# XUANTIE-RV/csi-nn2

Measured on AMD Instinct MI355X. Metric: mobilenetv1_int8_images_per_sec, higher is better.
Workload: dtype i8; 1 GPU; mobilenetv1 int8 NHWC batch 1/GPU, 28 conv layers in 15 launches, hipGraph replay via csinn_*; ops_per_image=1137480704, algorithmic_bytes_per_image=8323144, algorithmic_bytes_per_image_survey=14444616, parallelism=replicas x1

## Files before the change

csi-nn2_amd/csrc/conv1x1_latency.hip:

```cpp
#include <stdlib.h>

#include "igemm_common.h"

namespace shl {

struct LatPoolArgs {
    void *out;
    float si, zi, so, zo;
    int32_t store_map;
};

template <int NSW, int MT, int EPI, bool POOL>
__global__ __launch_bounds__(512) void conv1x1_latency_kernel(ConvArgs a, LatPoolArgs pl)
{
    extern __shared__ __attribute__((aligned(16))) char smem[];
    asm volatile("" ::"s"(a.in), "s"(a.w_frag), "s"(a.out), "s"(a.acc_init), "s"(a.mult), "s"(a.bias), "s"(a.C), "s"(a.Co), "s"(a.Ho), "s"(a.Wo));
    const int tid = threadIdx.x;
    const int lane = tid & 63;
    const int wave = __builtin_amdgcn_readfirstlane(tid >> 6);
    const int frow = lane & 31, fhalf = lane >> 5;
    const int slice = blockIdx.x, n = blockIdx.y;
    const int t0 = blockIdx.z;
    const int HW = a.Ho * a.Wo;
    constexpr int NSUB = 8 * NSW;
    const int sub0 = wave * NSW;

    const char *wp = static_cast<const char *>(a.w_frag) + ((int64_t)slice * NSUB + sub0) * 1024 + lane * 16;
    v4i fa[NSW];
#pragma unroll
    for (int s = 0; s < NSW; ++s) fa[s] = *reinterpret_cast<const v4i *>(wp + s * 1024);
    const char *img = static_cast<const char *>(a.in) + (int64_t)n * HW * a.C + fhalf * 16 + sub0 * 32;
    v4i fb[MT][NSW];
#pragma unroll
    for (int t = 0; t < MT; ++t) {
        const int p = min((t0 + t) * 32 + frow, HW - 1);
        const char *px = img + p * a.C;
#pragma unroll
        for (int s = 0; s < NSW; ++s) fb[t][s] = *reinterpret_cast<const v4i *>(px + s * 32);
    }
    const int fgrp = wave & 3, ftile = wave >> 2;
    const int pc = slice * 32 + 8 * fgrp + 4 * fhalf;
    const int4 p_ai = *reinterpret_cast<const int4 *>(a.acc_init + pc);
    const float4 p_mu = *reinterpret_cast<const float4 *>(a.mult + pc);
    const float4 p_bi = *reinterpret_cast<const float4 *>(a.bias + pc);

    const v16i zero16 = {0, 0, 0, 0, 0, 0, 0, 0, 0, 0, 0, 0, 0, 0, 0, 0};
    v16i acc[MT];
#pragma unroll
    for (int s = 0; s < NSW; ++s)
#pragma unroll
        for (int t = 0; t < MT; ++t) acc[t] = __builtin_amdgcn_mfma_i32_32x32x32_i8(fa[s], fb[t][s], s == 0 ? zero16 : acc[t], 0, 0, 0);

    v4i *part = reinterpret_cast<v4i *>(smem);
#pragma unroll
    for (int t = 0; t < MT; ++t)
#pragma unroll
        for (int g = 0; g < 4; ++g) {
            v4i v;
#pragma unroll
            for (int e = 0; e < 4; ++e) v[e] = acc[t][4 * g + e];
            part[((t * 8 + wave) * 4 + g) * 64 + lane] = v;
        }
    __syncthreads();
    uint32_t *pmap = reinterpret_cast<uint32_t *>(smem + (size_t)MT * 8 * 4096);
    if (ftile < MT) {
        v4i v = part[((ftile * 8) * 4 + fgrp) * 64 + lane];
#pragma unroll
        for (int k = 1; k < 8; ++k) v += part[((ftile * 8 + k) * 4 + fgrp) * 64 + lane];
        const uint32_t pk = requant4_i8_sel<EPI>(v[0] + p_ai.x, v[1] + p_ai.y, v[2] + p_ai.z, v[3] + p_ai.w, p_mu, p_bi, a);
        const int p = (t0 + ftile) * 32 + frow;
        if (p < HW) {
            if (!POOL || pl.store_map) *reinterpret_cast<uint32_t *>(static_cast<char *>(a.out) + ((int64_t)n * HW + p) * a.Co + pc) = pk;
            if constexpr (POOL) pmap[p * 8 + 2 * fgrp + fhalf] = pk;
        }
    }
    if constexpr (POOL) {
        __syncthreads();
        if (tid < 32) {
            const int8_t *col = reinterpret_cast<const int8_t *>(pmap) + tid;
            float total = 0.f;
            for (int p = 0; p < HW; ++p) total = __fadd_rn(total, __fmul_rn(__fsub_rn((float)col[p * 32], pl.zi), pl.si));
            const int q = sat8_from_float(__fadd_rn(rintf(__fdiv_rn(__fdiv_rn(total, (float)HW), pl.so)), pl.zo));
            static_cast<int8_t *>(pl.out)[(int64_t)n * a.Co + slice * 32 + tid] = (int8_t)q;
        }
    }
}

static int lat_epi(const ConvArgs &a) { return (a.act != SHL_MI355X_ACT_NONE && !a.act_clamp) ? -1 : (a.div_exact ? 3 : 0); }

static bool lat_shape(const ConvArgs &a)
{
    if (a.Kh != 1 || a.Kw != 1 || a.sh != 1 || a.sw != 1 || a.pt != 0 || a.pl != 0 || a.H != a.Ho || a.W != a.Wo) return false;
    if (a.C != 256 && a.C != 512 && a.C != 1024) return false;
    if ((a.Co & 31) != 0 || a.kstride < a.C || a.out_nchw || a.in_nchw || !a.w_frag) return false;
    const int HW = a.Ho * a.Wo;
    return HW >= 1 && HW <= 64 && a.N >= 1 && a.N <= 65535 && (a.Co >> 5) <= 65535;
}

bool conv1x1_latency_pick(const ConvArgs &a)
{
    if (!lat_shape(a)) return false;
    const char *env = getenv("SHL_MI355X_PWLAT");
    if (env && env[0] == '0') return false;
    if (env && env[0] == '1') return true;
    return (int64_t)(a.Co >> 5) * a.N <= 256;
}

bool conv1x1_pool_fusable(const ConvArgs &a) { return lat_shape(a) && (int64_t)(a.Co >> 5) * a.N <= 512; }

static int launch_lat(const ConvArgs &a, const LatPoolArgs &pl, hipStream_t s)
{
    const int HW = a.Ho * a.Wo, nsw = a.C / 256, epi = lat_epi(a);
    const bool pool = pl.out != nullptr;
    int mt = HW > 32 ? 2 : 1, zsplit = 1;
    const char *sp = getenv("SHL_MI355X_PWLAT_SPLIT");
    if (!pool && mt == 2 && (int64_t)(a.Co >> 5) * a.N * 2 <= 256 && !(sp && sp[0] == '0')) mt = 1, zsplit = 2;
    const dim3 grid((unsigned)(a.Co >> 5), (unsigned)a.N, (unsigned)zsplit);
    const size_t lds = (size_t)mt * 8 * 4096 + (pool ? (size_t)HW * 32 : 0);
#define SHL_LAT4(NSWV, MTV, EPIV, POOLV)                                                                      \
    do {                                                                                                      \
        static LdsOptIn opted;                                                                                \
        if (lds > 64 * 1024) lds_opt_in(opted, reinterpret_cast<const void *>(conv1x1_latency_kernel<NSWV, MTV, EPIV, POOLV>)); \
        hipLaunchKernelGGL((conv1x1_latency_kernel<NSWV, MTV, EPIV, POOLV>), grid, dim3(512), lds, s, a, pl);     \
    } while (0)
#define SHL_LAT3(NSWV, MTV, EPIV)             \
    do {                                      \
        if (pool) SHL_LAT4(NSWV, MTV, EPIV, true); \
        else SHL_LAT4(NSWV, MTV, EPIV, false);     \
    } while (0)
#define SHL_LAT2(NSWV, MTV)                    \
    do {                                       \
        if (epi == 3) SHL_LAT3(NSWV, MTV, 3);  \
        else if (epi == 0) SHL_LAT3(NSWV, MTV, 0); \
        else SHL_LAT3(NSWV, MTV, -1);          \
    } while (0)
#define SHL_LAT1(NSWV)               \
    do {                             \
        if (mt == 2) SHL_LAT2(NSWV, 2); \
        else SHL_LAT2(NSWV, 1);      \
    } while (0)
    if (nsw == 4) SHL_LAT1(4);
    else if (nsw == 2) SHL_LAT1(2);
    else SHL_LAT1(1);
#undef SHL_LAT1
#undef SHL_LAT2
#undef SHL_LAT3
#undef SHL_LAT4
    SHL_HIP(hipGetLastError());
    return SHL_MI355X_OK;
}

int launch_conv1x1_latency(const ConvArgs &a, hipStream_t s)
{
    if (!lat_shape(a)) {
        set_error("conv1x1_latency: the layer does not qualify");
        return SHL_MI355X_ENOTSUP;
    }
    LatPoolArgs pl = {};
    return launch_lat(a, pl, s);
}

int launch_conv1x1_pool(const ConvArgs &a, void *pool_out, float si, float zi, float so, float zo, int store_map, hipStream_t s)
{
    if (!conv1x1_pool_fusable(a) || !pool_out) {
        set_error("conv1x1_pool: the pair does not qualify");
        return SHL_MI355X_ENOTSUP;
// ... 8 lines not shown
```

csi-nn2_amd/csrc/conv_gemv.hip:

```cpp
#include <stdlib.h>

#include "common.h"

namespace shl {

constexpr int GEMV_OPW = 4;

template <bool kI8, int OPW>
__global__ __launch_bounds__(256) void conv_gemv_kernel(ConvArgs a)
{
    constexpr int ESIZE = kI8 ? 1 : 2;
    const int lane = threadIdx.x & 63;
    const int wave = __builtin_amdgcn_readfirstlane(threadIdx.x >> 6);
    const int p = blockIdx.y;
    const int oc0 = (blockIdx.x * 4 + wave) * OPW;
    if (oc0 >= a.Co) return;
    const int kb = a.C * ESIZE;
    const char *in = static_cast<const char *>(a.in) + (int64_t)p * kb;
    const char *w = static_cast<const char *>(a.w);
    int32_t acc_i[OPW];
    float acc_f[OPW];
#pragma unroll
    for (int o = 0; o < OPW; ++o) acc_i[o] = 0, acc_f[o] = 0.f;
    for (int off = lane * 16; off < kb; off += 1024) {
        const v4i x = *reinterpret_cast<const v4i *>(in + off);
        v4i wv[OPW];
#pragma unroll
        for (int o = 0; o < OPW; ++o) {
            const int oc = oc0 + o < a.Co ? oc0 + o : a.Co - 1;
            wv[o] = *reinterpret_cast<const v4i *>(w + (int64_t)oc * a.kstride + off);
        }
#pragma unroll
        for (int o = 0; o < OPW; ++o)
#pragma unroll
            for (int d = 0; d < 4; ++d) {
                if constexpr (kI8) {
                    acc_i[o] = __builtin_amdgcn_sdot4(x[d], wv[o][d], acc_i[o], false);
                } else {
                    const uint32_t xu = (uint32_t)x[d], wu = (uint32_t)wv[o][d];
                    acc_f[o] += f16_bits_to_float((uint16_t)(xu & 0xffffu)) * f16_bits_to_float((uint16_t)(wu & 0xffffu));
                    acc_f[o] += f16_bits_to_float((uint16_t)(xu >> 16)) * f16_bits_to_float((uint16_t)(wu >> 16));
                }
            }
    }
#pragma unroll
    for (int o = 0; o < OPW; ++o)
#pragma unroll
        for (int s = 32; s >= 1; s >>= 1) {
            if constexpr (kI8)
                acc_i[o] += __shfl_xor(acc_i[o], s, 64);
            else
                acc_f[o] += __shfl_xor(acc_f[o], s, 64);
        }
    if (lane < OPW && oc0 + lane < a.Co) {
        const int oc = oc0 + lane;
        int32_t S = acc_i[0];
        float F = acc_f[0];
#pragma unroll
        for (int o = 1; o < OPW; ++o) S = lane == o ? acc_i[o] : S, F = lane == o ? acc_f[o] : F;
        if constexpr (kI8) {
            static_cast<int8_t *>(a.out)[(int64_t)p * a.Co + oc] =
                (int8_t)requant_i8_fast(S + a.acc_init[oc], a.mult[oc], a.bias[oc], a);
        } else {
            static_cast<uint16_t *>(a.out)[(int64_t)p * a.Co + oc] = finish_f16(F, a.bias[oc], a);
        }
    }
}

constexpr int PG_WAVES = 16;

template <int QMAX>
__global__ __launch_bounds__(PG_WAVES * 64) void pool_gemv_i8_kernel(ConvArgs a, int HW, float si, float zi, float so, float zo)
{
    extern __shared__ __attribute__((aligned(16))) char x_lds[];
    const int tid = threadIdx.x, lane = tid & 63;
    const int wave = __builtin_amdgcn_readfirstlane(tid >> 6);
    const int p = blockIdx.y;
    const int oc0 = (blockIdx.x * PG_WAVES + wave) * GEMV_OPW;
    const bool live = oc0 < a.Co;
    const int kb = a.C;
    const char *w = static_cast<const char *>(a.w);
    v4i wv0[GEMV_OPW];
    {
        const int off = lane * 16;
#pragma unroll
        for (int o = 0; o < GEMV_OPW; ++o) {
            const int oc = oc0 + o < a.Co ? oc0 + o : a.Co - 1;
            wv0[o] = v4i{0, 0, 0, 0};
            if (off < kb) wv0[o] = *reinterpret_cast<const v4i *>(w + (int64_t)oc * a.kstride + off);
        }
    }
    const int row_b = a.C;
    const __amdgpu_buffer_rsrc_t img = __builtin_amdgcn_make_buffer_rsrc(
        const_cast<char *>(static_cast<const char *>(a.in) + (int64_t)p * HW * row_b), 0, HW * row_b, 0x00020000);
    for (int c = tid; c < a.C; c += PG_WAVES * 64) {
        uint32_t v[QMAX];
#pragma unroll
        for (int q = 0; q < QMAX; ++q) {
            const int qq = q < HW ? q : HW - 1;
            v[q] = (uint32_t)__builtin_amdgcn_raw_buffer_load_b32(img, c & ~3, qq * row_b, 0);
        }
        const int sh = 8 * (c & 3);
        float total = 0.f;
#pragma unroll
        for (int q = 0; q < QMAX; ++q) {
            const float x = __fmul_rn(__fsub_rn((float)(int8_t)(v[q] >> sh), zi), si);
            const float t = __fadd_rn(total, x);
            total = q < HW ? t : total;
        }
        x_lds[c] = (char)sat8_from_float(__fadd_rn(rintf(__fdiv_rn(__fdiv_rn(total, (float)HW), so)), zo));
    }
    __syncthreads();
    if (!live) return;
    int32_t acc_i[GEMV_OPW] = {0, 0, 0, 0};
    for (int off = lane * 16; off < kb; off += 1024) {
        const v4i x = *reinterpret_cast<const v4i *>(x_lds + off);
        v4i wv[GEMV_OPW];
#pragma unroll
        for (int o = 0; o < GEMV_OPW; ++o) {
            if (off < 1024) {
                wv[o] = wv0[o];
            } else {
                const int oc = oc0 + o < a.Co ? oc0 + o : a.Co - 1;
                wv[o] = *reinterpret_cast<const v4i *>(w + (int64_t)oc * a.kstride + off);
            }
        }
#pragma unroll
        for (int o = 0; o < GEMV_OPW; ++o)
#pragma unroll
            for (int d = 0; d < 4; ++d) acc_i[o] = __builtin_amdgcn_sdot4(x[d], wv[o][d], acc_i[o], false);
    }
#pragma unroll
    for (int o = 0; o < GEMV_OPW; ++o)
#pragma unroll
        for (int s = 32; s >= 1; s >>= 1) acc_i[o] += __shfl_xor(acc_i[o], s, 64);
    if (lane < GEMV_OPW && oc0 + lane < a.Co) {
        const int oc = oc0 + lane;
        const int32_t S = lane == 0 ? acc_i[0] : lane == 1 ? acc_i[1] : lane == 2 ? acc_i[2] : acc_i[3];
        static_cast<int8_t *>(a.out)[(int64_t)p * a.Co + oc] = (int8_t)requant_i8_fast(S + a.acc_init[oc], a.mult[oc], a.bias[oc], a);
    }
}

bool pool_gemv_pick(const ConvArgs &a, int hw)
{
    return conv_gemv_pick(a, 1) && a.H * a.W == 1 && hw >= 1 && hw <= 64 && a.C % 16 == 0 && a.C <= 32768 && (int64_t)hw * a.C < (1ll << 31);
}

// ... 36 lines not shown
```

csi-nn2_amd/csrc/dw_patch.h:

```cpp
#pragma once

#include "common.h"

namespace shl {

__device__ __forceinline__ int dw_patch_slot(int j, int group, int pitch) { return group * pitch + j; }
__host__ __device__ __forceinline__ int dw_patch_pitch(int npx) { return ((npx + 31) & ~31) + 8; }
__host__ __device__ __forceinline__ size_t dw_patch_bytes(int npx) { return (size_t)dw_patch_pitch(npx) * 32; }
__device__ __forceinline__ uint32_t dw_patch_pad(const ConvArgs &d) { return (uint32_t)(d.in_zp & 0xff) * 0x01010101u; }

struct DwPatchGeom {
    int bh, bw;
    int rw;
    int pitch;
    uint32_t bw_magic;
    int oy0, ox0;
    int ry0, rx0;
    int n;
    int ch0;
};

struct DwThreadConsts {
    uint4 w0, w1, w2;
    int4 ai;
    float4 mu, bi;
};

__device__ __forceinline__ DwThreadConsts dw_load_consts(const ConvArgs &d, int ch0, int tid)
{
    const int dc = ch0 + (tid & 7) * 4;
    const uint4 *dwp = reinterpret_cast<const uint4 *>(static_cast<const char *>(d.w) + (int64_t)dc * 12);
    DwThreadConsts k;
    k.w0 = dwp[0], k.w1 = dwp[1], k.w2 = dwp[2];
    k.ai = *reinterpret_cast<const int4 *>(d.acc_init + dc);
    k.mu = *reinterpret_cast<const float4 *>(d.mult + dc);
    k.bi = *reinterpret_cast<const float4 *>(d.bias + dc);
    return k;
}

template <int EPI = -1>
__device__ __forceinline__ void depthwise_from_patch(const ConvArgs &d, const uint32_t *patch, const DwPatchGeom &g,
                                                     const DwThreadConsts &k, int tid, int threads)
{
    const int cg = tid & 7;
    const int dc = g.ch0 + cg * 4;
    const uint4 w0 = k.w0, w1 = k.w1, w2 = k.w2;
    const int4 d_ai = k.ai;
    const float4 d_mu = k.mu, d_bi = k.bi;
    const uint32_t wk[12] = {w0.x, w0.y, w0.z, w0.w, w1.x, w1.y, w1.z, w1.w, w2.x, w2.y, w2.z, w2.w};
    const int nout = g.bh * g.bw;
    int8_t *const out_img = static_cast<int8_t *>(d.out) + (int64_t)g.n * d.Ho * d.Wo * d.C;
    for (int po = tid >> 3; po < nout; po += threads >> 3) {
        const int oyl = (int)(((uint32_t)po * g.bw_magic) >> 20);
        const int oxl = po - oyl * g.bw;
        const int oy = g.oy0 + oyl, ox = g.ox0 + oxl;
        if (oy >= d.Ho || ox >= d.Wo) continue;
        uint32_t iv[9];
        const uint32_t *p00 = patch + cg * g.pitch + (oyl * d.sh) * g.rw + oxl * d.sw;
#pragma unroll
        for (int ky = 0; ky < 3; ++ky)
#pragma unroll
            for (int kx = 0; kx < 3; ++kx) iv[ky * 3 + kx] = p00[ky * g.rw + kx];
        const uint32_t r0[4] = {iv[0], iv[1], iv[2], iv[3]}, r1[4] = {iv[4], iv[5], iv[6], iv[7]};
        uint32_t t0[4], t1[4];
        transpose4x4_bytes(r0, t0);
        transpose4x4_bytes(r1, t1);
        int a4[4] = {d_ai.x, d_ai.y, d_ai.z, d_ai.w};
#pragma unroll
        for (int ch = 0; ch < 4; ++ch) {
            const uint32_t t2 = __builtin_amdgcn_ubfe(iv[8], 8 * ch, 8);
            a4[ch] = __builtin_amdgcn_sdot4((int)t0[ch], (int)wk[3 * ch + 0], a4[ch], false);
            a4[ch] = __builtin_amdgcn_sdot4((int)t1[ch], (int)wk[3 * ch + 1], a4[ch], false);
            a4[ch] = __builtin_amdgcn_sdot4((int)t2, (int)wk[3 * ch + 2], a4[ch], false);
        }
        const uint32_t o = (uint32_t)((oy * d.Wo + ox) * d.C + dc);
        *reinterpret_cast<uint32_t *>(out_img + o) = requant4_i8_sel<EPI>(a4[0], a4[1], a4[2], a4[3], d_mu, d_bi, d);
    }
}

}
```

csi-nn2_amd/csrc/pwdw_fused.hip:

```cpp
#include <stdio.h>
#include <stdlib.h>

#include "dw_patch.h"
#include "igemm_common.h"

namespace shl {

struct PwDwArgs {
    ConvArgs pw;
    ConvArgs dw;
    int32_t bh, bw;
    int32_t tiles_x, tiles_y;
    int32_t rw;
    int32_t npx;
    int32_t mt;
    int32_t nwaves;
    int32_t ks;
    int32_t nsw;
    int32_t nsub;
    uint32_t rw_magic;
    uint32_t bw_magic;
    int32_t xg, xg_log2;
    int32_t spg;
    uint32_t spg_magic;
    uint32_t tx_magic;
    int32_t nrect;
    int32_t ks_log2;
    int32_t mwn;
    int64_t img_stride;
};

template <int MTW, int NSW, int MAXT, bool EXACT, int KSV = 0, int TPW = 0, bool EMT = false, int EPQ = -1, int EPD = -1>
__global__ __launch_bounds__(MAXT) void pwdw_fused_kernel(PwDwArgs f)
{
    static_assert((KSV == 0) == (TPW == 0) && (TPW == 0 || (TPW == MTW && EXACT)), "pwdw_fused: KSV and TPW come together, with MTW = TPW");
    constexpr bool FIXED = TPW != 0;
    extern __shared__ __attribute__((aligned(16))) char smem[];
    const ConvArgs &q = f.pw;
    const ConvArgs &d = f.dw;
    const int tid = threadIdx.x;
    const int lane = tid & 63;
    const int wave = __builtin_amdgcn_readfirstlane(tid >> 6);
    const int frow = lane & 31, fhalf = lane >> 5;
    asm volatile("" ::"s"(f.xg), "s"(f.xg_log2), "s"(f.spg), "s"(f.spg_magic), "s"(f.tx_magic), "s"(f.nrect), "s"(f.tiles_x), "s"(f.tiles_y));
    asm volatile("" ::"s"(f.bh), "s"(f.bw), "s"(f.rw), "s"(f.npx), "s"(f.mt), "s"(f.ks), "s"(f.nsw), "s"(f.nsub), "s"(f.rw_magic),
                 "s"(f.ks_log2), "s"(f.mwn), "s"(f.img_stride));
    asm volatile("" ::"s"(q.in), "s"(q.w_frag), "s"(q.H), "s"(q.W), "s"(q.C), "s"(d.sh), "s"(d.sw), "s"(d.pt), "s"(d.pl), "s"(d.N));
    int slice = blockIdx.x, tx = blockIdx.y, ty = blockIdx.z, n = 0;
    {
        const int L = blockIdx.x;
        const int x = L & 7, j = L >> 3;
        const int b = (int)(((uint32_t)j * f.spg_magic) >> 20);
        const int xslice = (x & (f.xg - 1)) * f.spg + (j - b * f.spg);
        const int rect = b * (8 >> f.xg_log2) + (x >> f.xg_log2);
        const int xty = (int)(((uint32_t)rect * f.tx_magic) >> 20);
        const int xtx = rect - xty * f.tiles_x;
        const bool mapped = f.xg != 0;
        if (mapped && rect >= f.nrect) return;
        slice = mapped ? xslice : slice;
        ty = mapped ? xty : ty;
        tx = mapped ? xtx : tx;
    }
    if (d.N > 1) {
        n = ty / f.tiles_y;
        ty -= n * f.tiles_y;
    }
    const int oy0 = ty * f.bh, ox0 = tx * f.bw;
    const int ry0 = oy0 * d.sh - d.pt, rx0 = ox0 * d.sw - d.pl;

    const int nwaves = FIXED ? 4 : f.nwaves;
    const int fgrp = wave & 3;

    const int ks = FIXED ? KSV : f.ks;
    const int kpart = wave & (ks - 1);
    const int mw = wave >> (FIXED ? (KSV == 4 ? 2 : (KSV == 2 ? 1 : 0)) : f.ks_log2);
    const int mwn = FIXED ? 4 / (KSV ? KSV : 1) : f.mwn;
    const int mtp = FIXED ? TPW * (4 / (KSV ? KSV : 1)) : f.mt;
    const int mt = (FIXED && EMT) ? mtp : f.mt;
    const int sub0 = kpart * f.nsw;
    int nsw = NSW;
    if constexpr (!EXACT) {
        nsw = f.nsub - sub0;
        nsw = nsw < f.nsw ? nsw : f.nsw;
    }

    const char *img = static_cast<const char *>(q.in) + (n ? (int64_t)n * f.img_stride : (int64_t)0);
    const char *wp = static_cast<const char *>(q.w_frag) + ((int64_t)slice * f.nsub + sub0) * 1024 + lane * 16;
    constexpr int wstep = 1024;
    v4i fa[NSW];
#pragma unroll
    for (int s = 0; s < NSW; ++s)
        if (s < nsw) fa[s] = *reinterpret_cast<const v4i *>(wp + s * wstep);
    v4i fb[MTW][NSW];
#pragma unroll
    for (int i = 0; i < MTW; ++i) {
        const int tile = mw + i * mwn;
        if (FIXED || tile < mt) {
            int j = tile * 32 + frow;
            j = j < f.npx ? j : f.npx - 1;
            const int r = (int)(((uint32_t)j * f.rw_magic) >> 20);
            const int c = j - r * f.rw;
            int y = ry0 + r, x = rx0 + c;
            y = max(0, min(y, q.H - 1));
            x = max(0, min(x, q.W - 1));
            const char *px = img + (y * q.W + x) * q.C + fhalf * 16 + sub0 * 32;
#pragma unroll
            for (int s = 0; s < NSW; ++s)
                if (s < nsw) fb[i][s] = *reinterpret_cast<const v4i *>(px + s * 32);
        }
    }
    const int pc = slice * 32 + 8 * fgrp + 4 * fhalf;
    const int4 p_ai = *reinterpret_cast<const int4 *>(q.acc_init + pc);
    const float4 p_mu = *reinterpret_cast<const float4 *>(q.mult + pc);
    const float4 p_bi = *reinterpret_cast<const float4 *>(q.bias + pc);

    const DwThreadConsts dwk = dw_load_consts(d, slice * 32, tid);

    v16i acc[MTW];
    if constexpr (EXACT) {
        const v16i zero16 = {0, 0, 0, 0, 0, 0, 0, 0, 0, 0, 0, 0, 0, 0, 0, 0};
#pragma unroll
        for (int s = 0; s < NSW; ++s) {
#pragma unroll
            for (int i = 0; i < MTW; ++i)
                if (FIXED || mw + i * mwn < mt) acc[i] = __builtin_amdgcn_mfma_i32_32x32x32_i8(fa[s], fb[i][s], s == 0 ? zero16 : acc[i], 0, 0, 0);
        }
    } else {
#pragma unroll
        for (int i = 0; i < MTW; ++i)
#pragma unroll
            for (int r = 0; r < 16; ++r) acc[i][r] = 0;
#pragma unroll
        for (int s = 0; s < NSW; ++s) {
            if (s < nsw) {
#pragma unroll
                for (int i = 0; i < MTW; ++i)
                    if (mw + i * mwn < mt) acc[i] = __builtin_amdgcn_mfma_i32_32x32x32_i8(fa[s], fb[i][s], acc[i], 0, 0, 0);
            }
        }
    }

    if (q.debug & 256) return;
    v4i *part = reinterpret_cast<v4i *>(smem);
    uint32_t *patch = reinterpret_cast<uint32_t *>(smem + (size_t)mtp * ks * 4096);
#pragma unroll
    for (int i = 0; i < MTW; ++i) {
        const int tile = mw + i * mwn;
        if (FIXED || tile < mt) {
#pragma unroll
            for (int g = 0; g < 4; ++g) {
                v4i v;
#pragma unroll
                for (int e = 0; e < 4; ++e) v[e] = acc[i][4 * g + e];
                part[((tile * ks + kpart) * 4 + g) * 64 + lane] = v;
            }
        }
    }
    __syncthreads();
    if (q.debug & 512) return;
    {
        const int ppitch = dw_patch_pitch(f.npx);
        const uint32_t zpad = dw_patch_pad(d);
        auto in_image = [&](int j) {
            const int r = (int)(((uint32_t)j * f.rw_magic) >> 20);
            const int c = j - r * f.rw;
            return (unsigned)(ry0 + r) < (unsigned)q.H && (unsigned)(rx0 + c) < (unsigned)q.W;
        };
        const int tstep = nwaves >> 2;
        for (int tile = FIXED ? 0 : wave >> 2; tile < mt; tile += 2 * tstep) {
            const int tile1 = tile + tstep;
            const int j0 = tile * 32 + frow;
            v4i v0 = part[((tile * ks) * 4 + fgrp) * 64 + lane];
            if (tile1 < mt) {
                v4i v1 = part[((tile1 * ks) * 4 + fgrp) * 64 + lane];
#pragma unroll
                for (int k = 1; k < ks; ++k) {
                    v0 += part[((tile * ks + k) * 4 + fgrp) * 64 + lane];
                    v1 += part[((tile1 * ks + k) * 4 + fgrp) * 64 + lane];
                }
                const uint32_t pk0 = requant4_i8_sel<EPQ>(v0[0] + p_ai.x, v0[1] + p_ai.y, v0[2] + p_ai.z, v0[3] + p_ai.w, p_mu, p_bi, q);
                const uint32_t pk1 = requant4_i8_sel<EPQ>(v1[0] + p_ai.x, v1[1] + p_ai.y, v1[2] + p_ai.z, v1[3] + p_ai.w, p_mu, p_bi, q);
                const int j1 = tile1 * 32 + frow;
                if (j0 < f.npx) patch[dw_patch_slot(j0, 2 * fgrp + fhalf, ppitch)] = in_image(j0) ? pk0 : zpad;
                if (j1 < f.npx) patch[dw_patch_slot(j1, 2 * fgrp + fhalf, ppitch)] = in_image(j1) ? pk1 : zpad;
            } else {
#pragma unroll
                for (int k = 1; k < ks; ++k) v0 += part[((tile * ks + k) * 4 + fgrp) * 64 + lane];
                const uint32_t pk0 = requant4_i8_sel<EPQ>(v0[0] + p_ai.x, v0[1] + p_ai.y, v0[2] + p_ai.z, v0[3] + p_ai.w, p_mu, p_bi, q);
                if (j0 < f.npx) patch[dw_patch_slot(j0, 2 * fgrp + fhalf, ppitch)] = in_image(j0) ? pk0 : zpad;
            }
        }
    }
    __syncthreads();

    if (q.debug & 1024) return;
    DwPatchGeom g;
    g.bh = f.bh, g.bw = f.bw, g.rw = f.rw, g.bw_magic = f.bw_magic, g.pitch = dw_patch_pitch(f.npx);
    g.oy0 = oy0, g.ox0 = ox0, g.ry0 = ry0, g.rx0 = rx0, g.n = n, g.ch0 = slice * 32;
    depthwise_from_patch<EPD>(d, patch, g, dwk, tid, nwaves * 64);
}

static int waves_per_group() { return 4; }
static int ks_for(int nsub, int nwaves)
{
    (void)nwaves;
    return nsub >= 8 ? 4 : (nsub >= 4 ? 2 : 1);
}
constexpr int PWDW_MTW = 4;

static bool shapes_pair(const ConvArgs &q, const ConvArgs &d)
{
    if (q.Kh != 1 || q.Kw != 1 || q.sh != 1 || q.sw != 1 || q.pt != 0 || q.pl != 0) return false;
    if (q.H != q.Ho || q.W != q.Wo || (q.C & 31) != 0 || (q.Co & 31) != 0 || q.kstride < q.C) return false;
    if (d.Kh != 3 || d.Kw != 3 || d.dh != 1 || d.dw != 1 || d.C != d.Co || d.C != q.Co) return false;
    if (d.H != q.Ho || d.W != q.Wo || d.N != q.N) return false;
    if (d.sh < 1 || d.sh > 2 || d.sw < 1 || d.sw > 2 || d.pt > 2 || d.pl > 2 || d.pt < 0 || d.pl < 0) return false;
    if (q.C > 1024 || !q.w_frag) return false;
    if ((int64_t)q.H * q.W * q.C >= ((int64_t)1 << 31)) return false;
    if ((int64_t)d.Ho * d.Wo * d.C >= ((int64_t)1 << 31)) return false;
    return true;
}

static bool choose_rect(const ConvArgs &q, const ConvArgs &d, PwDwArgs &f)
{
    const int nsub = q.C >> 5;
    const int nwaves = waves_per_group();
    const int ks = ks_for(nsub, nwaves);
    const int mt_max = (nwaves / ks) * PWDW_MTW;
    const int nsw = (nsub + ks - 1) / ks;
    if (nwaves == 8 && nsw > 4) return false;
    const int64_t slices = q.Co >> 5;
    int force_h = 0, force_w = 0;
    const char *env = getenv("SHL_MI355X_PWDW_TILE");
    if (env) sscanf(env, "%dx%d", &force_h, &force_w);
    double best = 1e30;
    int best_h = 0, best_w = 0;
    for (int bh = 1; bh <= d.Ho && bh <= 32; ++bh) {
        for (int div = 1; div <= 16; ++div) {
            const int bw = (d.Wo + div - 1) / div;
            if (div > 1 && bw == (d.Wo + div - 2) / (div - 1)) continue;
            if (force_h && (bh != force_h || bw != force_w)) continue;
            const int rh = (bh - 1) * d.sh + 3, rw = (bw - 1) * d.sw + 3;
            const int npx = rh * rw;
            const int mt = (npx + 31) / 32;
            if (mt > mt_max || rw > 256 || bw > 256 || npx >= 4096 || bh * bw >= 4096) continue;
            if ((size_t)mt * ks * 4096 + dw_patch_bytes(npx) > 96 * 1024) continue;
            const int64_t blocks = slices * ((d.Ho + bh - 1) / bh) * ((d.Wo + bw - 1) / bw) * d.N;
            const double rounds = (double)((blocks + 255) / 256);
            const double score = rounds * ((mt + 1) * nsub + 2.0 * ((bh * bw + 31) / 32) + 4.0) -
                                 (blocks <= 256 ? blocks / 1024.0 : 0.0);
            if (score < best) {
                best = score;
                best_h = bh;
                best_w = bw;
            }
        }
    }
    if (!best_h) return false;
    f.bh = best_h;
    f.bw = best_w;
    f.tiles_y = (d.Ho + f.bh - 1) / f.bh;
    f.tiles_x = (d.Wo + f.bw - 1) / f.bw;
    f.rw = (f.bw - 1) * d.sw + 3;
    f.npx = ((f.bh - 1) * d.sh + 3) * f.rw;
    f.mt = (f.npx + 31) / 32;
    f.nwaves = nwaves;
    f.ks = ks;
    f.nsw = nsw;
    f.nsub = nsub;
    f.ks_log2 = ks == 8 ? 3 : (ks == 4 ? 2 : (ks == 2 ? 1 : 0));
    f.mwn = nwaves / ks;
    f.img_stride = (int64_t)q.H * q.W * q.C;
    f.rw_magic = ((1u << 20) + f.rw - 1) / f.rw;
    f.bw_magic = ((1u << 20) + f.bw - 1) / f.bw;
    {
        const int S = (int)slices;
        const int64_t R = (int64_t)f.tiles_x * f.tiles_y * d.N;
        static const char *xe = getenv("SHL_MI355X_PWDW_XG");
        const int forced = xe ? atoi(xe) : -1;
        const double act = (double)q.N * q.H * q.W * q.C, wts = (double)q.C * q.Co;
        int best_g = 0;
        double best_c = 1e30;
// ... 116 lines not shown
```

csi-nn2_amd/csrc/stemdw_fused.hip:

```cpp
#include <stdio.h>
#include <stdlib.h>

#include "dw_patch.h"

namespace shl {

struct StemDwArgs {
    ConvArgs st;
    ConvArgs dw;
    int32_t bh, bw;
    int32_t tiles_x, tiles_y;
    int32_t rw, npx;
    uint32_t rw_magic, bw_magic;
};

template <int EPQ, int EPD>
__global__ __launch_bounds__(256) void stemdw_fused_kernel(StemDwArgs f)
{
    extern __shared__ __attribute__((aligned(16))) char smem[];
    const ConvArgs &q = f.st;
    const ConvArgs &d = f.dw;
    asm volatile("" ::"s"(q.in), "s"(q.w), "s"(q.acc_init), "s"(q.mult), "s"(q.bias), "s"(q.H), "s"(q.W), "s"(q.Ho), "s"(q.Wo), "s"(q.sh),
                 "s"(q.sw), "s"(q.pt), "s"(q.pl), "s"(q.dh), "s"(q.dw), "s"(q.in_zp));
    asm volatile("" ::"s"(f.bh), "s"(f.bw), "s"(f.tiles_y), "s"(f.rw), "s"(f.npx), "s"(f.rw_magic), "s"(f.bw_magic), "s"(d.N), "s"(d.sh),
                 "s"(d.sw), "s"(d.pt), "s"(d.pl), "s"(d.w), "s"(d.acc_init), "s"(d.mult), "s"(d.bias), "s"(d.out));
    asm volatile("" ::"s"(q.out_zp), "s"(q.out_zp_f), "s"(q.clamp_lo), "s"(q.clamp_hi), "s"(d.out_zp), "s"(d.out_zp_f), "s"(d.clamp_lo),
                 "s"(d.clamp_hi), "s"(d.in_zp), "s"(d.Ho), "s"(d.Wo), "s"(d.H), "s"(d.W), "s"(d.C));
    const int tid = threadIdx.x;
    int32_t *w_lds = reinterpret_cast<int32_t *>(smem);
    int32_t *t_tab = w_lds + 7 * 32;
    uint32_t *patch = reinterpret_cast<uint32_t *>(t_tab + 96);
    if (tid < 224) w_lds[tid] = static_cast<const int32_t *>(q.w)[tid];
    if (tid < 96) {
        const int which = tid >> 5, i = tid & 31;
        t_tab[tid] = which == 0 ? q.acc_init[i] : which == 1 ? __float_as_int(q.mult[i]) : __float_as_int(q.bias[i]);
    }
    const int tx = blockIdx.x;
    int ty = blockIdx.y, n = 0;
    if (d.N > 1) {
        n = ty / f.tiles_y;
        ty -= n * f.tiles_y;
    }
    const int oy0 = ty * f.bh, ox0 = tx * f.bw;
    const int ry0 = oy0 * d.sh - d.pt, rx0 = ox0 * d.sw - d.pl;
    const DwThreadConsts dwk = dw_load_consts(d, 0, tid);

    const int8_t *img = static_cast<const int8_t *>(q.in) + (int64_t)n * q.H * q.W * 3;
    const int ntasks = 2 * f.npx;
    const int ppitch = dw_patch_pitch(f.npx);
    const uint32_t zpad = dw_patch_pad(d);
    for (int base = 0; base < ntasks; base += 256) {
        const bool valid = base + tid < ntasks;
        const int task = valid ? base + tid : ntasks - 1;
        const int j = task >> 1, cb = (task & 1) * 16;
        const int pr = (int)(((uint32_t)j * f.rw_magic) >> 20);
        const int pc = j - pr * f.rw;
        const int sy = ry0 + pr, sx = rx0 + pc;
        const bool inside = (unsigned)sy < (unsigned)q.Ho && (unsigned)sx < (unsigned)q.Wo;
        const int y0 = sy * q.sh - q.pt, x0 = sx * q.sw - q.pl;
        int qv[28];
#pragma unroll
        for (int ky = 0; ky < 3; ++ky)
#pragma unroll
            for (int kx = 0; kx < 3; ++kx) {
                const int y = y0 + ky * q.dh, x = x0 + kx * q.dw;
                const bool ok = inside && (unsigned)y < (unsigned)q.H && (unsigned)x < (unsigned)q.W;
                const int8_t *px = img + ((int64_t)y * q.W + x) * 3;
#pragma unroll
                for (int c = 0; c < 3; ++c) qv[(ky * 3 + kx) * 3 + c] = ok ? (int)px[c] : q.in_zp;
            }
        qv[27] = 0;
        uint32_t q4[7];
#pragma unroll
        for (int g = 0; g < 7; ++g)
            q4[g] = (uint32_t)(qv[4 * g] & 0xFF) | ((uint32_t)(qv[4 * g + 1] & 0xFF) << 8) |
                    ((uint32_t)(qv[4 * g + 2] & 0xFF) << 16) | ((uint32_t)(qv[4 * g + 3] & 0xFF) << 24);
        if (base == 0) __syncthreads();
        int acc[16];
#pragma unroll
        for (int e = 0; e < 16; ++e) acc[e] = 0;
#pragma unroll
        for (int g = 0; g < 7; ++g)
#pragma unroll
            for (int v = 0; v < 4; ++v) {
                const int4 w = *reinterpret_cast<const int4 *>(&w_lds[g * 32 + cb + 4 * v]);
                acc[4 * v + 0] = __builtin_amdgcn_sdot4((int)q4[g], w.x, acc[4 * v + 0], false);
                acc[4 * v + 1] = __builtin_amdgcn_sdot4((int)q4[g], w.y, acc[4 * v + 1], false);
                acc[4 * v + 2] = __builtin_amdgcn_sdot4((int)q4[g], w.z, acc[4 * v + 2], false);
                acc[4 * v + 3] = __builtin_amdgcn_sdot4((int)q4[g], w.w, acc[4 * v + 3], false);
            }
#pragma unroll
        for (int v = 0; v < 4; ++v) {
            const int c = cb + 4 * v;
            const int4 ai = *reinterpret_cast<const int4 *>(t_tab + c);
            const float4 mu = *reinterpret_cast<const float4 *>(t_tab + 32 + c);
            const float4 bi = *reinterpret_cast<const float4 *>(t_tab + 64 + c);
            const uint32_t pk = requant4_i8_sel<EPQ>(acc[4 * v] + ai.x, acc[4 * v + 1] + ai.y, acc[4 * v + 2] + ai.z,
                                               acc[4 * v + 3] + ai.w, mu, bi, q);
            if (valid) patch[dw_patch_slot(j, c >> 2, ppitch)] = inside ? pk : zpad;
        }
    }
    __syncthreads();

    DwPatchGeom g;
    g.bh = f.bh, g.bw = f.bw, g.rw = f.rw, g.bw_magic = f.bw_magic, g.pitch = ppitch;
    g.oy0 = oy0, g.ox0 = ox0, g.ry0 = ry0, g.rx0 = rx0, g.n = n, g.ch0 = 0;
    depthwise_from_patch<EPD>(d, patch, g, dwk, tid, 256);
}

static bool stemdw_geometry(const ConvArgs &q, const ConvArgs &d, StemDwArgs &f)
{
    if (q.Kh != 3 || q.Kw != 3 || q.C != 3 || q.Co != 32) return false;
    if (d.Kh != 3 || d.Kw != 3 || d.dh != 1 || d.dw != 1 || d.C != 32 || d.Co != 32) return false;
    if (d.H != q.Ho || d.W != q.Wo || d.N != q.N || d.sh < 1 || d.sh > 2 || d.sw < 1 || d.sw > 2) return false;
    if (d.pt < 0 || d.pl < 0 || d.pt > 2 || d.pl > 2) return false;
    if ((int64_t)d.Ho * d.Wo * d.C >= ((int64_t)1 << 31)) return false;
    f.bh = d.Ho < 2 ? d.Ho : 2;
    f.bw = d.Wo < 28 ? d.Wo : 28;
    if (const char *e = getenv("SHL_MI355X_STEMDW_TILE")) {
        int h = 0, w = 0;
        if (sscanf(e, "%dx%d", &h, &w) == 2 && h > 0 && w > 0) f.bh = h < d.Ho ? h : d.Ho, f.bw = w < d.Wo ? w : d.Wo;
    }
    f.tiles_y = (d.Ho + f.bh - 1) / f.bh;
    f.tiles_x = (d.Wo + f.bw - 1) / f.bw;
    f.rw = (f.bw - 1) * d.sw + 3;
    f.npx = ((f.bh - 1) * d.sh + 3) * f.rw;
    f.rw_magic = ((1u << 20) + f.rw - 1) / f.rw;
    f.bw_magic = ((1u << 20) + f.bw - 1) / f.bw;
    if (f.npx >= 2048 || f.tiles_x > 65535 || (int64_t)f.tiles_y * d.N > 65535) return false;
    return (int64_t)f.tiles_x * f.tiles_y * d.N <= 2048;
}

bool stemdw_fusable(const ConvArgs &q, const ConvArgs &d)
{
    StemDwArgs f;
    return stemdw_geometry(q, d, f);
}

int launch_stemdw_fused(const ConvArgs &q, const ConvArgs &d, hipStream_t s)
{
    StemDwArgs f;
    f.st = q;
    f.dw = d;
    if (!stemdw_geometry(q, d, f)) {
        set_error("stemdw_fused: the pair does not qualify");
        return SHL_MI355X_ENOTSUP;
    }
    const dim3 grid((unsigned)f.tiles_x, (unsigned)(f.tiles_y * d.N));
    const size_t lds = (size_t)(7 * 32 + 96) * 4 + dw_patch_bytes(f.npx);
    const int epq = (q.act != SHL_MI355X_ACT_NONE && !q.act_clamp) ? -1 : (q.div_exact ? 3 : 0);
    const int epd = (d.act != SHL_MI355X_ACT_NONE && !d.act_clamp) ? -1 : (d.div_exact ? 3 : 0);
    if (epq == 3 && epd == 3) hipLaunchKernelGGL((stemdw_fused_kernel<3, 3>), grid, dim3(256), lds, s, f);
    else if (epq == 0 && epd == 0) hipLaunchKernelGGL((stemdw_fused_kernel<0, 0>), grid, dim3(256), lds, s, f);
    else hipLaunchKernelGGL((stemdw_fused_kernel<-1, -1>), grid, dim3(256), lds, s, f);
    SHL_HIP(hipGetLastError());
    return SHL_MI355X_OK;
}

}
```

Baseline: 17590 img/s.

## Hoist kernarg, epilogue-constant and address setup ahead of MFMA in fused conv kernels

Reads the kernel arguments for the epilogue (quant params, clamp values, pool args) straight from the kernarg segment and forces them into scalar registers early. Sched barriers and empty asm pin these loads and the output-address and patch-slot math before the MFMA work, so their latency overlaps compute instead of stalling the epilogue. The depthwise-from-patch loop is restructured to precompute the first output position and compute the next position at the end of each iteration. It also hoists per-channel loads in the gemv kernel and removes debug early-return checks in the FIXED path. The cost is higher scalar and vector register pressure, and the forced barriers constrain the compiler's scheduling.

```diff
diff --git a/csi-nn2_amd/csrc/conv1x1_latency.hip b/csi-nn2_amd/csrc/conv1x1_latency.hip
--- a/csi-nn2_amd/csrc/conv1x1_latency.hip
+++ b/csi-nn2_amd/csrc/conv1x1_latency.hip
@@ -1,8 +1,20 @@
+#include <stddef.h>
 #include <stdlib.h>
 
 #include "igemm_common.h"
 
 namespace shl {
+
+template <class T>
+__device__ __forceinline__ T kernarg_here(size_t off)
+{
+    typedef const __attribute__((address_space(4))) char *KernargPtr;
+    KernargPtr p = (KernargPtr)__builtin_amdgcn_kernarg_segment_ptr();
+    asm volatile("" : "+s"(p));
+    T v;
+    __builtin_memcpy(&v, (const __attribute__((address_space(4))) T *)(p + off), sizeof(T));
+    return v;
+}
 
 struct LatPoolArgs {
     void *out;
@@ -29,6 +41,7 @@
     v4i fa[NSW];
 #pragma unroll
     for (int s = 0; s < NSW; ++s) fa[s] = *reinterpret_cast<const v4i *>(wp + s * 1024);
+    __builtin_amdgcn_sched_barrier(0);
     const char *img = static_cast<const char *>(a.in) + (int64_t)n * HW * a.C + fhalf * 16 + sub0 * 32;
     v4i fb[MT][NSW];
 #pragma unroll
@@ -38,11 +51,26 @@
 #pragma unroll
         for (int s = 0; s < NSW; ++s) fb[t][s] = *reinterpret_cast<const v4i *>(px + s * 32);
     }
+    __builtin_amdgcn_sched_barrier(0);
+    const ConvArgs al = kernarg_here<ConvArgs>(0);
+    const LatPoolArgs pll = kernarg_here<LatPoolArgs>((sizeof(ConvArgs) + alignof(LatPoolArgs) - 1) & ~(alignof(LatPoolArgs) - 1));
+    asm volatile("" ::"s"(al.out_zp), "s"(al.out_zp_f), "s"(al.clamp_lo), "s"(al.clamp_hi), "s"(al.out_scale), "s"(al.inv_out_scale), "s"(al.act),
+                 "s"(al.div_exact));
+    if constexpr (POOL) asm volatile("" ::"s"(pll.out), "s"(pll.si), "s"(pll.zi), "s"(pll.so), "s"(pll.zo), "s"(pll.store_map));
     const int fgrp = wave & 3, ftile = wave >> 2;
     const int pc = slice * 32 + 8 * fgrp + 4 * fhalf;
     const int4 p_ai = *reinterpret_cast<const int4 *>(a.acc_init + pc);
     const float4 p_mu = *reinterpret_cast<const float4 *>(a.mult + pc);
     const float4 p_bi = *reinterpret_cast<const float4 *>(a.bias + pc);
+    const int fp = (t0 + ftile) * 32 + frow;
+    uint32_t *const fout = reinterpret_cast<uint32_t *>(static_cast<char *>(a.out) + ((int64_t)n * HW + fp) * a.Co + pc);
+    const uint32_t fslot = (uint32_t)(fp * 8 + 2 * fgrp + fhalf);
+    {
+        const float cl = al.clamp_lo - al.out_zp_f, ch = al.clamp_hi - al.out_zp_f;
+        const uint32_t zp2 = (uint32_t)(al.out_zp & 0xffff) * 0x00010001u;
+        asm volatile("" ::"v"(fp), "v"(fout), "v"(fslot), "v"(cl), "v"(ch), "s"(zp2));
+    }
+    __builtin_amdgcn_sched_barrier(0);
 
     const v16i zero16 = {0, 0, 0, 0, 0, 0, 0, 0, 0, 0, 0, 0, 0, 0, 0, 0};
     v16i acc[MT];
@@ -67,11 +95,10 @@
         v4i v = part[((ftile * 8) * 4 + fgrp) * 64 + lane];
 #pragma unroll
         for (int k = 1; k < 8; ++k) v += part[((ftile * 8 + k) * 4 + fgrp) * 64 + lane];
-        const uint32_t pk = requant4_i8_sel<EPI>(v[0] + p_ai.x, v[1] + p_ai.y, v[2] + p_ai.z, v[3] + p_ai.w, p_mu, p_bi, a);
-        const int p = (t0 + ftile) * 32 + frow;
-        if (p < HW) {
-            if (!POOL || pl.store_map) *reinterpret_cast<uint32_t *>(static_cast<char *>(a.out) + ((int64_t)n * HW + p) * a.Co + pc) = pk;
-            if constexpr (POOL) pmap[p * 8 + 2 * fgrp + fhalf] = pk;
+        const uint32_t pk = requant4_i8_sel<EPI>(v[0] + p_ai.x, v[1] + p_ai.y, v[2] + p_ai.z, v[3] + p_ai.w, p_mu, p_bi, al);
+        if (fp < HW) {
+            if (!POOL || pll.store_map) *fout = pk;
+            if constexpr (POOL) pmap[fslot] = pk;
         }
     }
     if constexpr (POOL) {
@@ -79,9 +106,9 @@
         if (tid < 32) {
             const int8_t *col = reinterpret_cast<const int8_t *>(pmap) + tid;
             float total = 0.f;
-            for (int p = 0; p < HW; ++p) total = __fadd_rn(total, __fmul_rn(__fsub_rn((float)col[p * 32], pl.zi), pl.si));
-            const int q = sat8_from_float(__fadd_rn(rintf(__fdiv_rn(__fdiv_rn(total, (float)HW), pl.so)), pl.zo));
-            static_cast<int8_t *>(pl.out)[(int64_t)n * a.Co + slice * 32 + tid] = (int8_t)q;
+            for (int p = 0; p < HW; ++p) total = __fadd_rn(total, __fmul_rn(__fsub_rn((float)col[p * 32], pll.zi), pll.si));
+            const int q = sat8_from_float(__fadd_rn(rintf(__fdiv_rn(__fdiv_rn(total, (float)HW), pll.so)), pll.zo));
+            static_cast<int8_t *>(pll.out)[(int64_t)n * a.Co + slice * 32 + tid] = (int8_t)q;
         }
     }
 }
diff --git a/csi-nn2_amd/csrc/conv_gemv.hip b/csi-nn2_amd/csrc/conv_gemv.hip
--- a/csi-nn2_amd/csrc/conv_gemv.hip
+++ b/csi-nn2_amd/csrc/conv_gemv.hip
@@ -10,6 +10,9 @@
 __global__ __launch_bounds__(256) void conv_gemv_kernel(ConvArgs a)
 {
     constexpr int ESIZE = kI8 ? 1 : 2;
+    asm volatile("" ::"s"(a.in), "s"(a.w), "s"(a.out), "s"(a.acc_init), "s"(a.mult), "s"(a.bias), "s"(a.C), "s"(a.Co), "s"(a.kstride));
+    asm volatile("" ::"s"(a.out_zp_f), "s"(a.clamp_lo), "s"(a.clamp_hi), "s"(a.act), "s"(a.act_clamp), "s"(a.div_exact), "s"(a.out_scale),
+                 "s"(a.inv_out_scale), "s"(a.scale_out));
     const int lane = threadIdx.x & 63;
     const int wave = __builtin_amdgcn_readfirstlane(threadIdx.x >> 6);
     const int p = blockIdx.y;
@@ -22,6 +25,11 @@
     float acc_f[OPW];
 #pragma unroll
     for (int o = 0; o < OPW; ++o) acc_i[o] = 0, acc_f[o] = 0.f;
+    const int oc = oc0 + lane < a.Co ? oc0 + lane : a.Co - 1;
+    int32_t e_ai = 0;
+    float e_mu = 0.f;
+    if constexpr (kI8) e_ai = a.acc_init[oc], e_mu = a.mult[oc];
+    const float e_bi = a.bias[oc];
     for (int off = lane * 16; off < kb; off += 1024) {
         const v4i x = *reinterpret_cast<const v4i *>(in + off);
         v4i wv[OPW];
@@ -53,16 +61,14 @@
                 acc_f[o] += __shfl_xor(acc_f[o], s, 64);
         }
     if (lane < OPW && oc0 + lane < a.Co) {
-        const int oc = oc0 + lane;
         int32_t S = acc_i[0];
         float F = acc_f[0];
 #pragma unroll
         for (int o = 1; o < OPW; ++o) S = lane == o ? acc_i[o] : S, F = lane == o ? acc_f[o] : F;
         if constexpr (kI8) {
-            static_cast<int8_t *>(a.out)[(int64_t)p * a.Co + oc] =
-                (int8_t)requant_i8_fast(S + a.acc_init[oc], a.mult[oc], a.bias[oc], a);
+            static_cast<int8_t *>(a.out)[(int64_t)p * a.Co + oc] = (int8_t)requant_i8_fast(S + e_ai, e_mu, e_bi, a);
         } else {
-            static_cast<uint16_t *>(a.out)[(int64_t)p * a.Co + oc] = finish_f16(F, a.bias[oc], a);
+            static_cast<uint16_t *>(a.out)[(int64_t)p * a.Co + oc] = finish_f16(F, e_bi, a);
         }
     }
 }
diff --git a/csi-nn2_amd/csrc/dw_patch.h b/csi-nn2_amd/csrc/dw_patch.h
--- a/csi-nn2_amd/csrc/dw_patch.h
+++ b/csi-nn2_amd/csrc/dw_patch.h
@@ -1,4 +1,6 @@
 #pragma once
+
+#include <stddef.h>
 
 #include "common.h"
 
@@ -8,6 +10,17 @@
 __host__ __device__ __forceinline__ int dw_patch_pitch(int npx) { return ((npx + 31) & ~31) + 8; }
 __host__ __device__ __forceinline__ size_t dw_patch_bytes(int npx) { return (size_t)dw_patch_pitch(npx) * 32; }
 __device__ __forceinline__ uint32_t dw_patch_pad(const ConvArgs &d) { return (uint32_t)(d.in_zp & 0xff) * 0x01010101u; }
+
+template <class T>
+__device__ __forceinline__ T kernarg_here(size_t off)
+{
+    typedef const __attribute__((address_space(4))) char *KernargPtr;
+    KernargPtr p = (KernargPtr)__builtin_amdgcn_kernarg_segment_ptr();
+    asm volatile("" : "+s"(p));
+    T v;
+    __builtin_memcpy(&v, (const __attribute__((address_space(4))) T *)(p + off), sizeof(T));
+    return v;
+}
 
 struct DwPatchGeom {
     int bh, bw;
@@ -38,43 +51,81 @@
     return k;
 }
 
+struct DwOutPos {
+    uint32_t lds;
+    uint32_t out;
+    bool live;
+};
+
+struct DwPrep {
+    int8_t *out_img;
+    int nout;
+    int po;
+    DwOutPos first;
+};
+
+__device__ __forceinline__ DwOutPos dw_patch_locate(const ConvArgs &d, const DwPatchGeom &g, int cg, int po)
+{
+    const int oyl = (int)(((uint32_t)po * g.bw_magic) >> 20);
+    const int oxl = po - oyl * g.bw;
+    const int oy = g.oy0 + oyl, ox = g.ox0 + oxl;
+    DwOutPos p;
+    p.lds = (uint32_t)(cg * g.pitch + (oyl * d.sh) * g.rw + oxl * d.sw);
+    p.out = (uint32_t)((oy * d.Wo + ox) * d.C + g.ch0 + cg * 4);
+    p.live = oy < d.Ho && ox < d.Wo;
+    return p;
+}
+
+__device__ __forceinline__ DwPrep dw_patch_prepare(const ConvArgs &d, const DwPatchGeom &g, int tid)
+{
+    DwPrep p;
+    p.out_img = static_cast<int8_t *>(d.out) + (g.n ? (int64_t)g.n * d.Ho * d.Wo * d.C : (int64_t)0);
+    p.nout = g.bh * g.bw;
+    p.po = tid >> 3;
+    p.first = dw_patch_locate(d, g, tid & 7, p.po);
+    const uint32_t live = p.first.live ? 1u : 0u;
+    asm volatile("" ::"s"(p.out_img), "s"(p.nout), "v"(p.po), "v"(p.first.lds), "v"(p.first.out), "v"(live));
+    p.first.live = live != 0;
+    return p;
+}
+
 template <int EPI = -1>
 __device__ __forceinline__ void depthwise_from_patch(const ConvArgs &d, const uint32_t *patch, const DwPatchGeom &g,
-                                                     const DwThreadConsts &k, int tid, int threads)
+                                                     const DwThreadConsts &k, const DwPrep &prep, int tid, int threads)
 {
     const int cg = tid & 7;
-    const int dc = g.ch0 + cg * 4;
     const uint4 w0 = k.w0, w1 = k.w1, w2 = k.w2;
     const int4 d_ai = k.ai;
     const float4 d_mu = k.mu, d_bi = k.bi;
     const uint32_t wk[12] = {w0.x, w0.y, w0.z, w0.w, w1.x, w1.y, w1.z, w1.w, w2.x, w2.y, w2.z, w2.w};
-    const int nout = g.bh * g.bw;
-    int8_t *const out_img = static_cast<int8_t *>(d.out) + (int64_t)g.n * d.Ho * d.Wo * d.C;
-    for (int po = tid >> 3; po < nout; po += threads >> 3) {
-        const int oyl = (int)(((uint32_t)po * g.bw_magic) >> 20);
-        const int oxl = po - oyl * g.bw;
-        const int oy = g.oy0 + oyl, ox = g.ox0 + oxl;
-        if (oy >= d.Ho || ox >= d.Wo) continue;
-        uint32_t iv[9];
-        const uint32_t *p00 = patch + cg * g.pitch + (oyl * d.sh) * g.rw + oxl * d.sw;
+    const int nout = prep.nout;
+    int8_t *const out_img = prep.out_img;
+    DwOutPos pos = prep.first;
+    for (int po = prep.po; po < nout;) {
+        const DwOutPos cur = pos;
+        if (cur.live) {
+            uint32_t iv[9];
+            const uint32_t *p00 = patch + cur.lds;
 #pragma unroll
-        for (int ky = 0; ky < 3; ++ky)
+            for (int ky = 0; ky < 3; ++ky)
 #pragma unroll
-            for (int kx = 0; kx < 3; ++kx) iv[ky * 3 + kx] = p00[ky * g.rw + kx];
-        const uint32_t r0[4] = {iv[0], iv[1], iv[2], iv[3]}, r1[4] = {iv[4], iv[5], iv[6], iv[7]};
-        uint32_t t0[4], t1[4];
-        transpose4x4_bytes(r0, t0);
-        transpose4x4_bytes(r1, t1);
-        int a4[4] = {d_ai.x, d_ai.y, d_ai.z, d_ai.w};
+                for (int kx = 0; kx < 3; ++kx) iv[ky * 3 + kx] = p00[ky * g.rw + kx];
+            const uint32_t r0[4] = {iv[0], iv[1], iv[2], iv[3]}, r1[4] = {iv[4], iv[5], iv[6], iv[7]};
+            uint32_t t0[4], t1[4];
+            transpose4x4_bytes(r0, t0);
+            transpose4x4_bytes(r1, t1);
+            int a4[4] = {d_ai.x, d_ai.y, d_ai.z, d_ai.w};
 #pragma unroll
-        for (int ch = 0; ch < 4; ++ch) {
-            const uint32_t t2 = __builtin_amdgcn_ubfe(iv[8], 8 * ch, 8);
-            a4[ch] = __builtin_amdgcn_sdot4((int)t0[ch], (int)wk[3 * ch + 0], a4[ch], false);
-            a4[ch] = __builtin_amdgcn_sdot4((int)t1[ch], (int)wk[3 * ch + 1], a4[ch], false);
-            a4[ch] = __builtin_amdgcn_sdot4((int)t2, (int)wk[3 * ch + 2], a4[ch], false);
+            for (int ch = 0; ch < 4; ++ch) {
+                const uint32_t t2 = __builtin_amdgcn_ubfe(iv[8], 8 * ch, 8);
+                a4[ch] = __builtin_amdgcn_sdot4((int)t0[ch], (int)wk[3 * ch + 0], a4[ch], false);
+                a4[ch] = __builtin_amdgcn_sdot4((int)t1[ch], (int)wk[3 * ch + 1], a4[ch], false);
+                a4[ch] = __builtin_amdgcn_sdot4((int)t2, (int)wk[3 * ch + 2], a4[ch], false);
+            }
+            *reinterpret_cast<uint32_t *>(out_img + cur.out) = requant4_i8_sel<EPI>(a4[0], a4[1], a4[2], a4[3], d_mu, d_bi, d);
         }
-        const uint32_t o = (uint32_t)((oy * d.Wo + ox) * d.C + dc);
-        *reinterpret_cast<uint32_t *>(out_img + o) = requant4_i8_sel<EPI>(a4[0], a4[1], a4[2], a4[3], d_mu, d_bi, d);
+        po += threads >> 3;
+        pos = dw_patch_locate(d, g, cg, po);
     }
 }
 
diff --git a/csi-nn2_amd/csrc/pwdw_fused.hip b/csi-nn2_amd/csrc/pwdw_fused.hip
--- a/csi-nn2_amd/csrc/pwdw_fused.hip
+++ b/csi-nn2_amd/csrc/pwdw_fused.hip
@@ -91,6 +91,7 @@
 #pragma unroll
     for (int s = 0; s < NSW; ++s)
         if (s < nsw) fa[s] = *reinterpret_cast<const v4i *>(wp + s * wstep);
+    if constexpr (FIXED) __builtin_amdgcn_sched_barrier(0);
     v4i fb[MTW][NSW];
 #pragma unroll
     for (int i = 0; i < MTW; ++i) {
@@ -109,12 +110,47 @@
                 if (s < nsw) fb[i][s] = *reinterpret_cast<const v4i *>(px + s * 32);
         }
     }
+    __builtin_amdgcn_sched_barrier(0);
+    const uint32_t bw_magic = kernarg_here<uint32_t>(offsetof(PwDwArgs, bw_magic));
+    const ConvArgs ql = kernarg_here<ConvArgs>(offsetof(PwDwArgs, pw)), dl = kernarg_here<ConvArgs>(offsetof(PwDwArgs, dw));
+    asm volatile("" ::"s"(ql.acc_init), "s"(ql.mult), "s"(ql.bias), "s"(ql.out_zp), "s"(ql.out_zp_f), "s"(ql.clamp_lo), "s"(ql.clamp_hi),
+                 "s"(ql.out_scale), "s"(ql.inv_out_scale), "s"(dl.w), "s"(dl.acc_init), "s"(dl.mult), "s"(dl.bias), "s"(dl.out));
+    asm volatile("" ::"s"(dl.out_zp), "s"(dl.out_zp_f), "s"(dl.clamp_lo), "s"(dl.clamp_hi), "s"(dl.out_scale), "s"(dl.inv_out_scale),
+                 "s"(dl.in_zp), "s"(dl.Ho), "s"(dl.Wo), "s"(dl.C), "s"(dl.sh), "s"(dl.sw), "s"(bw_magic));
     const int pc = slice * 32 + 8 * fgrp + 4 * fhalf;
-    const int4 p_ai = *reinterpret_cast<const int4 *>(q.acc_init + pc);
-    const float4 p_mu = *reinterpret_cast<const float4 *>(q.mult + pc);
-    const float4 p_bi = *reinterpret_cast<const float4 *>(q.bias + pc);
-
-    const DwThreadConsts dwk = dw_load_consts(d, slice * 32, tid);
+    const int4 p_ai = *reinterpret_cast<const int4 *>(ql.acc_init + pc);
+    const float4 p_mu = *reinterpret_cast<const float4 *>(ql.mult + pc);
+    const float4 p_bi = *reinterpret_cast<const float4 *>(ql.bias + pc);
+
+    const DwThreadConsts dwk = dw_load_consts(dl, slice * 32, tid);
+    DwPatchGeom g;
+    g.bh = f.bh, g.bw = f.bw, g.rw = f.rw, g.bw_magic = bw_magic, g.pitch = dw_patch_pitch(f.npx);
+    g.oy0 = oy0, g.ox0 = ox0, g.ry0 = ry0, g.rx0 = rx0, g.n = n, g.ch0 = slice * 32;
+    const DwPrep dwp = dw_patch_prepare(dl, g, tid);
+    const int ppitch = g.pitch;
+    const uint32_t zpad = dw_patch_pad(dl);
+    {
+        const float qcl = ql.clamp_lo - ql.out_zp_f, qch = ql.clamp_hi - ql.out_zp_f, dcl = dl.clamp_lo - dl.out_zp_f, dch = dl.clamp_hi - dl.out_zp_f;
+        const uint32_t qzp2 = (uint32_t)(ql.out_zp & 0xffff) * 0x00010001u, dzp2 = (uint32_t)(dl.out_zp & 0xffff) * 0x00010001u;
+        asm volatile("" ::"s"(ppitch), "s"(zpad), "v"(qcl), "v"(qch), "v"(dcl), "v"(dch), "s"(qzp2), "s"(dzp2));
+    }
+    auto in_image = [&](int j) {
+        const int r = (int)(((uint32_t)j * f.rw_magic) >> 20);
+        const int c = j - r * f.rw;
+        return (unsigned)(ry0 + r) < (unsigned)q.H && (unsigned)(rx0 + c) < (unsigned)q.W;
+    };
+    constexpr int NFT = (FIXED && EMT) ? TPW * (4 / (KSV ? KSV : 1)) : 1;
+    uint32_t fslot[NFT], fkeep[NFT];
+    if constexpr (FIXED && EMT) {
+#pragma unroll
+        for (int t = 0; t < NFT; ++t) {
+            const int j = t * 32 + frow;
+            fslot[t] = (uint32_t)dw_patch_slot(j, 2 * fgrp + fhalf, ppitch);
+            fkeep[t] = in_image(j) ? 0xffffffffu : 0u;
+            asm volatile("" ::"v"(fslot[t]), "v"(fkeep[t]));
+        }
+    }
+    __builtin_amdgcn_sched_barrier(0);
 
     v16i acc[MTW];
     if constexpr (EXACT) {
@@ -140,7 +176,8 @@
         }
     }
 
-    if (q.debug & 256) return;
+    if constexpr (!FIXED)
+        if (q.debug & 256) return;
     v4i *part = reinterpret_cast<v4i *>(smem);
     uint32_t *patch = reinterpret_cast<uint32_t *>(smem + (size_t)mtp * ks * 4096);
 #pragma unroll
@@ -157,14 +194,15 @@
         }
     }
     __syncthreads();
-    if (q.debug & 512) return;
+    if constexpr (!FIXED)
+        if (q.debug & 512) return;
     {
-        const int ppitch = dw_patch_pitch(f.npx);
-        const uint32_t zpad = dw_patch_pad(d);
-        auto in_image = [&](int j) {
-            const int r = (int)(((uint32_t)j * f.rw_magic) >> 20);
-            const int c = j - r * f.rw;
-            return (unsigned)(ry0 + r) < (unsigned)q.H && (unsigned)(rx0 + c) < (unsigned)q.W;
+        auto put = [&](int tile, int j, uint32_t pk) {
+            if constexpr (FIXED && EMT) {
+                if (j < f.npx) patch[fslot[tile]] = (pk & fkeep[tile]) | (zpad & ~fkeep[tile]);
+            } else {
+                if (j < f.npx) patch[dw_patch_slot(j, 2 * fgrp + fhalf, ppitch)] = in_image(j) ? pk : zpad;
+            }
         };
         const int tstep = nwaves >> 2;
         for (int tile = FIXED ? 0 : wave >> 2; tile < mt; tile += 2 * tstep) {
@@ -178,26 +216,24 @@
                     v0 += part[((tile * ks + k) * 4 + fgrp) * 64 + lane];
                     v1 += part[((tile1 * ks + k) * 4 + fgrp) * 64 + lane];
                 }
-                const uint32_t pk0 = requant4_i8_sel<EPQ>(v0[0] + p_ai.x, v0[1] + p_ai.y, v0[2] + p_ai.z, v0[3] + p_ai.w, p_mu, p_bi, q);
-                const uint32_t pk1 = requant4_i8_sel<EPQ>(v1[0] + p_ai.x, v1[1] + p_ai.y, v1[2] + p_ai.z, v1[3] + p_ai.w, p_mu, p_bi, q);
+                const uint32_t pk0 = requant4_i8_sel<EPQ>(v0[0] + p_ai.x, v0[1] + p_ai.y, v0[2] + p_ai.z, v0[3] + p_ai.w, p_mu, p_bi, ql);
+                const uint32_t pk1 = requant4_i8_sel<EPQ>(v1[0] + p_ai.x, v1[1] + p_ai.y, v1[2] + p_ai.z, v1[3] + p_ai.w, p_mu, p_bi, ql);
                 const int j1 = tile1 * 32 + frow;
-                if (j0 < f.npx) patch[dw_patch_slot(j0, 2 * fgrp + fhalf, ppitch)] = in_image(j0) ? pk0 : zpad;
-                if (j1 < f.npx) patch[dw_patch_slot(j1, 2 * fgrp + fhalf, ppitch)] = in_image(j1) ? pk1 : zpad;
+                put(tile, j0, pk0);
+                put(tile1, j1, pk1);
             } else {
 #pragma unroll
                 for (int k = 1; k < ks; ++k) v0 += part[((tile * ks + k) * 4 + fgrp) * 64 + lane];
-                const uint32_t pk0 = requant4_i8_sel<EPQ>(v0[0] + p_ai.x, v0[1] + p_ai.y, v0[2] + p_ai.z, v0[3] + p_ai.w, p_mu, p_bi, q);
-                if (j0 < f.npx) patch[dw_patch_slot(j0, 2 * fgrp + fhalf, ppitch)] = in_image(j0) ? pk0 : zpad;
+                const uint32_t pk0 = requant4_i8_sel<EPQ>(v0[0] + p_ai.x, v0[1] + p_ai.y, v0[2] + p_ai.z, v0[3] + p_ai.w, p_mu, p_bi, ql);
+                put(tile, j0, pk0);
             }
         }
     }
     __syncthreads();
 
-    if (q.debug & 1024) return;
-    DwPatchGeom g;
-    g.bh = f.bh, g.bw = f.bw, g.rw = f.rw, g.bw_magic = f.bw_magic, g.pitch = dw_patch_pitch(f.npx);
-    g.oy0 = oy0, g.ox0 = ox0, g.ry0 = ry0, g.rx0 = rx0, g.n = n, g.ch0 = slice * 32;
-    depthwise_from_patch<EPD>(d, patch, g, dwk, tid, nwaves * 64);
+    if constexpr (!FIXED)
+        if (q.debug & 1024) return;
+    depthwise_from_patch<EPD>(dl, patch, g, dwk, dwp, tid, nwaves * 64);
 }
 
 static int waves_per_group() { return 4; }
diff --git a/csi-nn2_amd/csrc/stemdw_fused.hip b/csi-nn2_amd/csrc/stemdw_fused.hip
--- a/csi-nn2_amd/csrc/stemdw_fused.hip
+++ b/csi-nn2_amd/csrc/stemdw_fused.hip
@@ -49,6 +49,10 @@
     const int ntasks = 2 * f.npx;
     const int ppitch = dw_patch_pitch(f.npx);
     const uint32_t zpad = dw_patch_pad(d);
+    DwPatchGeom g;
+    g.bh = f.bh, g.bw = f.bw, g.rw = f.rw, g.bw_magic = f.bw_magic, g.pitch = ppitch;
+    g.oy0 = oy0, g.ox0 = ox0, g.ry0 = ry0, g.rx0 = rx0, g.n = n, g.ch0 = 0;
+    const DwPrep dwp = dw_patch_prepare(d, g, tid);
     for (int base = 0; base < ntasks; base += 256) {
         const bool valid = base + tid < ntasks;
         const int task = valid ? base + tid : ntasks - 1;
@@ -102,10 +106,7 @@
     }
     __syncthreads();
 
-    DwPatchGeom g;
-    g.bh = f.bh, g.bw = f.bw, g.rw = f.rw, g.bw_magic = f.bw_magic, g.pitch = ppitch;
-    g.oy0 = oy0, g.ox0 = ox0, g.ry0 = ry0, g.rx0 = rx0, g.n = n, g.ch0 = 0;
-    depthwise_from_patch<EPD>(d, patch, g, dwk, tid, 256);
+    depthwise_from_patch<EPD>(d, patch, g, dwk, dwp, tid, 256);
 }
 
 static bool stemdw_geometry(const ConvArgs &q, const ConvArgs &d, StemDwArgs &f)
```

Result: faster. 18910 img/s, median of 6 (+7.5%).
